# giech/usrp_nfc

Hardware: NVIDIA B200
Metric: decoded_msamples_per_s (higher is better)
Workload: dtype f64

## Files before the change

usrp_nfc_b200/csrc/linecode.cu:

```cuda
#include "common.cuh"
#include "scan.cuh"

#include <algorithm>

namespace nfc {

#ifndef NFC_LC_CHUNK
#define NFC_LC_CHUNK 64
#endif
static const int CHUNK = NFC_LC_CHUNK;
static const int LOOKBACK_LIMIT = 4096;
static const int RSTATES = 32, GSTATES = 16;

struct __align__(16) ChunkMap {
    uint8_t r[RSTATES];
    uint8_t g[GSTATES];
};
struct ComposeMap {
    __device__ __forceinline__ ChunkMap operator()(const ChunkMap &a, const ChunkMap &b) const {
        ChunkMap c;
#pragma unroll
        for (int s = 0; s < RSTATES; s++) c.r[s] = b.r[a.r[s] & 31];
#pragma unroll
        for (int s = 0; s < GSTATES; s++) c.g[s] = b.g[a.g[s] & 15];
// ... 213 lines not shown
    maps[c] = m;
}

struct CountSink {
    ChunkCnt c;
    __device__ __forceinline__ void symbol(uint32_t, int, int) { c.nsym++; }
    __device__ __forceinline__ void emission(uint32_t, int type) {
        uint32_t &has = type == 0 ? c.has0 : c.has1;
        uint32_t &tail = type == 0 ? c.tail0 : c.tail1;
        if (tail != 0) c.nemit++;
        else if (!(has & 1)) { c.nemit++; has |= 2; }
        has |= 1;
        tail = 0;
    }
    __device__ __forceinline__ void bit(int type, int) {
        if (type == 0) { c.nbit0++; c.tail0++; } else { c.nbit1++; c.tail1++; }
    }
    __device__ __forceinline__ void new_capture() {
        c.has0 |= 1; c.tail0 = 0;
        c.has1 |= 1; c.tail1 = 0;
    }
};

__global__ void chunk_summary_kernel(const EventRec *__restrict__ ev, EvCount evc, LineTables lt,
                                     uint16_t *__restrict__ summary) {
    NFC_TABLE_SMEM
    const uint32_t c = blockIdx.x * blockDim.x + threadIdx.x;
    const uint32_t n_ev = evc.n(), n_chunks = (n_ev + CHUNK - 1) / CHUNK;
    if (c >= n_chunks) return;
    int rs = 0, gs = 0;
    bool kR = false, kG = false;
    NullSink sink;
    const uint32_t i0 = c * CHUNK, i1 = min(n_ev, i0 + CHUNK);
    uint32_t cap_prev = tv.pitch ? batch_capture_before(tv, ev, (int64_t)i0) : 0u;
    for (uint32_t i = i0; i < i1; i += 8) {
        EventRec e8[8];
        load8(ev, i, e8);
#pragma unroll
        for (int k = 0; k < 8; k++) {
            if (i + k >= i1) continue;
            const EventRec e = e8[k];
            int dummy = 0;
            if (tv.pitch) {
                bool inside;
                const uint32_t cap = batch_capture(tv, e.rel_pos, inside);
                if (cap != cap_prev) {
// ... 65 lines not shown
                }
                if (!inside) continue;
            }
            if (e.type == 1) {
                if (kk > iR) step_event(e, tv, rs, dummy_g, sink);
            } else if (e.type == 0) {
                if (kk > iG) step_event(e, tv, dummy_r, gs, sink);
            }
        }
    }
    start[c] = (uint16_t)(rs | (gs << 8));
}

__global__ void chunk_start_from_maps_kernel(const ChunkMap *__restrict__ prefix, const DecCarry *__restrict__ carry_in,
                                             uint16_t *__restrict__ start, uint32_t n_chunks) {
    const uint32_t c = blockIdx.x * blockDim.x + threadIdx.x;
    if (c >= n_chunks) return;
    const DecCarry carry = *carry_in;
    const int rs0 = (carry.miller_state & 15) | ((carry.started[1] & 1) << 4);
    const int gs0 = (carry.manch_state & 7) | ((carry.started[0] & 1) << 3);
    start[c] = (uint16_t)(prefix[c].r[rs0] | (prefix[c].g[gs0] << 8));
}

__global__ void chunk_count_kernel(const EventRec *__restrict__ ev, EvCount evc, LineTables lt,
                                   const uint16_t *__restrict__ start, ChunkCnt *__restrict__ cnts, uint32_t cap_chunks) {
    NFC_TABLE_SMEM
    const uint32_t c = blockIdx.x * blockDim.x + threadIdx.x;
    const uint32_t n_ev = evc.n(), n_chunks = (n_ev + CHUNK - 1) / CHUNK;
    if (c >= cap_chunks) return;
    CountSink sink;
    sink.c = ChunkCnt{0, 0, 0, 0, 0, 0, 0, 0};
    if (c >= n_chunks) {
        cnts[c] = sink.c;
        return;
    }
    int rs = start[c] & 31, gs = (start[c] >> 8) & 15;
    const uint32_t i0 = c * CHUNK, i1 = min(n_ev, i0 + CHUNK);
    uint32_t cap_prev = tv.pitch ? batch_capture_before(tv, ev, (int64_t)i0) : 0u;
    for (uint32_t i = i0; i < i1; i += 8) {
        EventRec e[8];
        load8(ev, i, e);
#pragma unroll
        for (int k = 0; k < 8; k++)
            if (i + k < i1) step_event_batch(e[k], tv, rs, gs, sink, cap_prev);
    }
    cnts[c] = sink.c;
}

struct WriteSink {
    SymbolRec *sym;
    uint8_t *bits0, *bits1;
    FrameRec *fr;
    unsigned long long *fx;
    uint32_t *n_empty;
    int64_t a;
    unsigned long long base0, base1;
    uint32_t isym, ib0, ib1, iem;
    uint32_t pend0, pend1;
    uint32_t cap_sym, cap_b0, cap_b1, cap_em;
    __device__ __forceinline__ void symbol(uint32_t pos, int type, int o) {
        if (sym && isym < cap_sym) {
            SymbolRec s;
            s.rel_pos = pos; s.type = (int8_t)type; s.val = (int8_t)o; s.pad = 0;
            sym[isym] = s;
        }
        isym++;
    }
    __device__ __forceinline__ void emission(uint32_t pos, int type) {
        const uint32_t nbits = type == 0 ? pend0 : pend1;
// ... 16 lines not shown
    }
    __device__ __forceinline__ void bit(int type, int o) {
        if (type == 0) { if (ib0 < cap_b0) bits0[ib0] = (uint8_t)o; ib0++; pend0++; }
        else { if (ib1 < cap_b1) bits1[ib1] = (uint8_t)o; ib1++; pend1++; }
    }
    __device__ __forceinline__ void new_capture() { pend0 = 0; pend1 = 0; }
};

struct LineOut {
    SymbolRec *sym;
    uint8_t *bits0, *bits1;
    FrameRec *fr;
    unsigned long long *fx;
    uint32_t cap_sym, cap_b0, cap_b1, cap_em;
    const uint32_t *pending_in;
    int64_t a;
    const unsigned long long *bits_in;
    unsigned long long *bits_out;
    uint32_t *n_empty;
    uint32_t *n_frames;
};

__global__ void chunk_write_kernel(const EventRec *__restrict__ ev, EvCount evc, LineTables lt,
                                   const uint16_t *__restrict__ start,
                                   const ChunkCnt *__restrict__ cnt_prefix, LineOut out, const DecCarry *__restrict__ carry_in,
                                   DecCarry *__restrict__ carry_out, uint32_t *__restrict__ pending_out) {
    NFC_TABLE_SMEM
    const uint32_t c = blockIdx.x * blockDim.x + threadIdx.x;
    const uint32_t n_ev = evc.n(), n_chunks = (n_ev + CHUNK - 1) / CHUNK;
    if (n_chunks == 0 && c == 0) {
        *carry_out = *carry_in;
        pending_out[0] = out.pending_in[0];
        pending_out[1] = out.pending_in[1];
        out.bits_out[0] = out.bits_in[0];
        out.bits_out[1] = out.bits_in[1];
    }
    if (c >= n_chunks) return;
    int rs = start[c] & 31, gs = (start[c] >> 8) & 15;
    const ChunkCnt pc = cnt_prefix[c];
    WriteSink sink;
    sink.sym = out.sym; sink.bits0 = out.bits0; sink.bits1 = out.bits1; sink.fr = out.fr; sink.fx = out.fx;
    sink.n_empty = out.n_empty; sink.a = out.a; sink.base0 = out.bits_in[0]; sink.base1 = out.bits_in[1];
    sink.cap_sym = out.cap_sym; sink.cap_b0 = out.cap_b0; sink.cap_b1 = out.cap_b1; sink.cap_em = out.cap_em;
    sink.isym = pc.nsym; sink.ib0 = pc.nbit0; sink.ib1 = pc.nbit1; sink.iem = resolved_records(pc, out.pending_in);
    sink.pend0 = (pc.has0 & 1) ? pc.tail0 : out.pending_in[0] + pc.tail0;
    sink.pend1 = (pc.has1 & 1) ? pc.tail1 : out.pending_in[1] + pc.tail1;
    const uint32_t i0 = c * CHUNK, i1 = min(n_ev, i0 + CHUNK);
    uint32_t cap_prev = tv.pitch ? batch_capture_before(tv, ev, (int64_t)i0) : 0u;
    for (uint32_t i = i0; i < i1; i += 8) {
        EventRec e[8];
        load8(ev, i, e);
#pragma unroll
        for (int k = 0; k < 8; k++)
            if (i + k < i1) step_event_batch(e[k], tv, rs, gs, sink, cap_prev);
    }
    if (c == n_chunks - 1) {
        DecCarry co;
        co.miller_state = rs & 15; co.started[1] = rs >> 4;
        co.manch_state = gs & 7; co.started[0] = gs >> 3;
        *carry_out = co;
        pending_out[0] = sink.pend0;
        pending_out[1] = sink.pend1;
        out.bits_out[0] = sink.base0 + sink.ib0;
        out.bits_out[1] = sink.base1 + sink.ib1;
        *out.n_frames = sink.iem;
    }
}

uint32_t linecode_chunks(uint32_t n_ev) { return (n_ev + CHUNK - 1) / CHUNK; }
size_t linecode_map_bytes() { return sizeof(ChunkMap); }
size_t linecode_cnt_bytes() { return sizeof(ChunkCnt); }
size_t linecode_emission_bytes() { return sizeof(FrameRec); }
size_t linecode_scratch_bytes(uint32_t n_chunks) {
    return scan_scratch_elems(n_chunks) * sizeof(ChunkMap) + scan_scratch_elems(n_chunks) * sizeof(ChunkCnt);
}

int launch_linecode_start(const EventRec *d_ev, const uint32_t *d_M, uint32_t cap_ev, const LineTables &lt, const DecCarry *d_carry_in,
                          uint16_t *d_summary, uint16_t *d_start, uint32_t *d_flags, cudaStream_t stream) {
    const uint32_t nc = std::max(1u, linecode_chunks(cap_ev));
    const EvCount evc{d_M, cap_ev};
    chunk_summary_kernel<<<(nc + 127) / 128, 128, 0, stream>>>(d_ev, evc, lt, d_summary);
    NFC_CUDA_CHECK(cudaGetLastError());
    chunk_start_kernel<<<(nc + 127) / 128, 128, 0, stream>>>(d_ev, evc, lt, d_carry_in, d_summary, d_start, d_flags);
    NFC_CUDA_CHECK(cudaGetLastError());
    return 0;
}

int launch_linecode_start_scan(const EventRec *d_ev, const uint32_t *d_M, uint32_t cap_ev, const LineTables &lt,
                               const DecCarry *d_carry_in, void *d_maps, void *d_prefix, void *d_scratch, uint16_t *d_start,
                               cudaStream_t stream) {
    const uint32_t nc = std::max(1u, linecode_chunks(cap_ev));
    ChunkMap *maps = (ChunkMap *)d_maps, *prefix = (ChunkMap *)d_prefix;
    const unsigned nb = (nc + 127) / 128;
    const EvCount evc{d_M, cap_ev};
    chunk_map_kernel<<<nb, 128, 0, stream>>>(d_ev, evc, lt, maps, nc);
    NFC_CUDA_CHECK(cudaGetLastError());
    ChunkMap ident;
    for (int s = 0; s < RSTATES; s++) ident.r[s] = (uint8_t)s;
    for (int s = 0; s < GSTATES; s++) ident.g[s] = (uint8_t)s;
    if (device_exclusive_scan<ChunkMap, ComposeMap>(maps, prefix, nc, ident, ComposeMap(), (ChunkMap *)d_scratch, nullptr, stream))
        return -1;
    chunk_start_from_maps_kernel<<<nb, 128, 0, stream>>>(prefix, d_carry_in, d_start, nc);
    NFC_CUDA_CHECK(cudaGetLastError());
    return 0;
}

int launch_linecode_count(const EventRec *d_ev, const uint32_t *d_M, uint32_t cap_ev, const LineTables &lt, const uint16_t *d_start,
                          void *d_cnts, void *d_cnt_prefix, void *d_scratch, void *d_total, cudaStream_t stream) {
    const uint32_t nc = std::max(1u, linecode_chunks(cap_ev));
    ChunkCnt *cnts = (ChunkCnt *)d_cnts, *cprefix = (ChunkCnt *)d_cnt_prefix;
    const EvCount evc{d_M, cap_ev};
    chunk_count_kernel<<<(nc + 127) / 128, 128, 0, stream>>>(d_ev, evc, lt, d_start, cnts, nc);
    NFC_CUDA_CHECK(cudaGetLastError());
    ChunkCnt zero = {0, 0, 0, 0, 0, 0, 0, 0};
    return device_exclusive_scan<ChunkCnt, CombineCnt>(cnts, cprefix, nc, zero, CombineCnt(), (ChunkCnt *)d_scratch,
                                                       (ChunkCnt *)d_total, stream);
}

int launch_linecode_write(const EventRec *d_ev, const uint32_t *d_M, uint32_t cap_ev, const LineTables &lt, const uint16_t *d_start,
                          const void *d_cnt_prefix, SymbolRec *d_sym, uint32_t cap_sym, uint8_t *d_bits0, uint32_t cap_b0,
                          uint8_t *d_bits1, uint32_t cap_b1, void *d_frames, void *d_findex, uint32_t cap_em, int64_t a,
                          const void *d_bits_in, void *d_bits_out, uint32_t *d_n_empty, uint32_t *d_n_frames, const uint32_t *d_pending_in,
                          const DecCarry *d_carry_in, DecCarry *d_carry_out, uint32_t *d_pending_out, cudaStream_t stream) {
    const uint32_t nc = std::max(1u, linecode_chunks(cap_ev));
    LineOut out;
    out.sym = d_sym; out.bits0 = d_bits0; out.bits1 = d_bits1; out.fr = (FrameRec *)d_frames; out.fx = (unsigned long long *)d_findex;
    out.cap_sym = cap_sym; out.cap_b0 = cap_b0; out.cap_b1 = cap_b1; out.cap_em = cap_em;
    out.pending_in = d_pending_in;
    out.a = a;
    out.bits_in = (const unsigned long long *)d_bits_in;
    out.bits_out = (unsigned long long *)d_bits_out;
    out.n_empty = d_n_empty;
    out.n_frames = d_n_frames;
    const EvCount evc{d_M, cap_ev};
    chunk_write_kernel<<<(nc + 127) / 128, 128, 0, stream>>>(d_ev, evc, lt, d_start, (const ChunkCnt *)d_cnt_prefix, out,
                                                             d_carry_in, d_carry_out, d_pending_out);
    NFC_CUDA_CHECK(cudaGetLastError());
    return 0;
}

}
```

usrp_nfc_b200/csrc/runs.cu:

```cuda
#include "common.cuh"
#include "scan.cuh"

namespace nfc {

__global__ void seg_offsets_kernel(const uint32_t *__restrict__ counts, uint32_t *__restrict__ offsets, int n) {
    __shared__ uint32_t sh[1024];
    __shared__ uint32_t carry;
    if (threadIdx.x == 0) carry = 0;
    __syncthreads();
    for (int base = 0; base < n; base += 1024) {
        const int i = base + threadIdx.x;
        uint32_t v = i < n ? counts[i] : 0u;
        sh[threadIdx.x] = v;
        __syncthreads();
        for (int o = 1; o < 1024; o <<= 1) {
            uint32_t a = threadIdx.x >= o ? sh[threadIdx.x - o] : 0u;
            __syncthreads();
            sh[threadIdx.x] += a;
            __syncthreads();
        }
        if (i < n) offsets[i] = carry + sh[threadIdx.x] - v;
        __syncthreads();
        if (threadIdx.x == 1023) carry += sh[1023];
        __syncthreads();
// ... 84 lines not shown
    }
}

struct RunArgs {
    const TransRec *tr;
    const uint32_t *d_R;
    uint32_t cap_R;
    int32_t w0, w1;
    const RunCarry *rc_in;
    int mx;
    uint32_t *flags;
};
__device__ __forceinline__ RunView make_view(const RunArgs &A) {
    RunView V;
    const RunCarry c = *A.rc_in;
    V.tr = A.tr;
    V.R = min(*A.d_R, A.cap_R);
    V.w0 = A.w0; V.w1 = A.w1;
    V.st0 = c.st; V.lb0 = c.last_bit; V.dur0 = c.dur;
    V.mx = A.mx;
    return V;
}

__global__ void run_count_kernel(RunArgs A, int keep_dropped, uint32_t *__restrict__ counts) {
    const uint32_t r = blockIdx.x * blockDim.x + threadIdx.x;
    if (r > A.cap_R) return;
    const RunView V = make_view(A);
    if (r == 0 && *A.d_R > A.cap_R) atomicOr(A.flags, (uint32_t)POST_OVF_TRANS);
    uint32_t c = 0;
    if (r <= V.R) run_events(V, r, keep_dropped != 0, [&](uint32_t, int, int, int) { c++; });
    counts[r] = c;
}

__global__ void run_write_kernel(RunArgs A, int keep_dropped, const uint32_t *__restrict__ offsets,
                                 EventRec *__restrict__ out, uint32_t cap, const uint32_t *__restrict__ d_M,
                                 RunCarry *__restrict__ carry_out) {
    const uint32_t r = blockIdx.x * blockDim.x + threadIdx.x;
    if (r > A.cap_R) return;
    const RunView V = make_view(A);
    if (r == 0 && *d_M > cap) atomicOr(A.flags, (uint32_t)POST_OVF_EVENTS);
    if (r > V.R) return;
    uint32_t idx = offsets[r];
    run_events(V, r, keep_dropped != 0, [&](uint32_t pos, int v, int d, int type) {
        if (idx < cap) {
            EventRec ev;
            ev.rel_pos = pos;
            ev.d = (uint16_t)d;
            ev.v = (int8_t)v;
            ev.type = (int8_t)type;
            out[idx] = ev;
        }
        idx++;
    });
    if (r == V.R && carry_out) {
        RunCarry c;
        if (V.w1 > V.w0) {
            c.st = V.s_end(r);
            c.last_bit = V.u(r);
            c.dur = (int)((uint32_t)(V.w1 - 1 - V.p(r)) % (uint32_t)V.mx) + 1;
        } else {
            c.st = V.st0; c.last_bit = V.lb0; c.dur = V.dur0;
        }
        c.pad = 0;
        *carry_out = c;
    }
}

int launch_gather_transitions(const SegWork *d_works, const uint32_t *d_counts, uint32_t *d_offsets, int n_segs,
                              TransRec *d_dense, cudaStream_t stream) {
    if (n_segs <= 0) return 0;
    seg_offsets_kernel<<<1, 1024, 0, stream>>>(d_counts, d_offsets, n_segs);
    NFC_CUDA_CHECK(cudaGetLastError());
    gather_trans_kernel<<<n_segs, 256, 0, stream>>>(d_works, d_counts, d_offsets, d_dense);
    NFC_CUDA_CHECK(cudaGetLastError());
    return 0;
}

int launch_gather_pieces(const TransRec *const *d_src, const uint32_t *d_n, const uint32_t *d_off, int n_pieces,
                         TransRec *d_dense, cudaStream_t stream) {
    if (n_pieces <= 0) return 0;
    gather_pieces_kernel<<<n_pieces, 256, 0, stream>>>(d_src, d_n, d_off, d_dense);
    NFC_CUDA_CHECK(cudaGetLastError());
    return 0;
}

int launch_run_count(const TransRec *d_tr, const uint32_t *d_R, uint32_t cap_R, int64_t w0, int64_t w1, const RunCarry *d_rc_in,
                     int mx, int keep_dropped, uint32_t *d_counts, uint32_t *d_offsets, uint32_t *d_scratch, uint32_t *d_total,
                     uint32_t *d_flags, cudaStream_t stream) {
    RunArgs A;
    A.tr = d_tr; A.d_R = d_R; A.cap_R = cap_R; A.w0 = (int32_t)w0; A.w1 = (int32_t)w1; A.rc_in = d_rc_in; A.mx = mx; A.flags = d_flags;
    const uint32_t nrun = cap_R + 1;
    run_count_kernel<<<(nrun + 255) / 256, 256, 0, stream>>>(A, keep_dropped, d_counts);
    NFC_CUDA_CHECK(cudaGetLastError());
    return device_exclusive_scan<uint32_t, AddU32>(d_counts, d_offsets, nrun, 0u, AddU32(), d_scratch, d_total, stream);
}

int launch_run_write(const TransRec *d_tr, const uint32_t *d_R, uint32_t cap_R, int64_t w0, int64_t w1, const RunCarry *d_rc_in,
                     int mx, int keep_dropped, const uint32_t *d_offsets, EventRec *d_events, uint32_t cap, const uint32_t *d_M,
                     RunCarry *d_carry_out, uint32_t *d_flags, cudaStream_t stream) {
    RunArgs A;
    A.tr = d_tr; A.d_R = d_R; A.cap_R = cap_R; A.w0 = (int32_t)w0; A.w1 = (int32_t)w1; A.rc_in = d_rc_in; A.mx = mx; A.flags = d_flags;
    const uint32_t nrun = cap_R + 1;
    run_write_kernel<<<(nrun + 255) / 256, 256, 0, stream>>>(A, keep_dropped, d_offsets, d_events, cap, d_M, d_carry_out);
    NFC_CUDA_CHECK(cudaGetLastError());
    return 0;
}

}
```

usrp_nfc_b200/csrc/scan.cuh:

```cuda
#pragma once

#include <cuda_runtime.h>

#include <vector>

#include "common.cuh"

namespace nfc {

static const int SCAN_BLOCK = 256;
static const int SCAN_ITEMS = 4;
static const int SCAN_TILE = SCAN_BLOCK * SCAN_ITEMS;

template <class T>
__device__ __forceinline__ T shfl_up_any(const T &v, int delta) {
    static_assert(sizeof(T) % 4 == 0, "T must be a multiple of 4 bytes");
    T r;
    const unsigned *src = reinterpret_cast<const unsigned *>(&v);
    unsigned *dst = reinterpret_cast<unsigned *>(&r);
#pragma unroll
    for (int i = 0; i < (int)(sizeof(T) / 4); i++) dst[i] = __shfl_up_sync(0xffffffffu, src[i], delta);
    return r;
}

// ... 59 lines not shown

template <class T, class Op>
int device_exclusive_scan(const T *in, T *out, size_t n, T identity, Op op, T *scratch, T *total_out,
                          cudaStream_t stream) {
    if (n == 0) {
        if (total_out) NFC_CUDA_CHECK(cudaMemcpyAsync(total_out, &identity, 0, cudaMemcpyHostToDevice, stream));
        return 0;
    }
    const size_t nb = scan_blocks(n);
    T *totals = scratch;
    T *totals_excl = scratch + nb;
    scan_block_kernel<T, Op><<<(unsigned)nb, SCAN_BLOCK, 0, stream>>>(in, out, totals, n, identity, op);
    NFC_CUDA_CHECK(cudaGetLastError());
    if (nb == 1) {
        if (total_out) NFC_CUDA_CHECK(cudaMemcpyAsync(total_out, totals, sizeof(T), cudaMemcpyDeviceToDevice, stream));
        return 0;
    }
    if (device_exclusive_scan<T, Op>(totals, totals_excl, nb, identity, op, scratch + 2 * nb, total_out, stream)) return -1;
    scan_add_kernel<T, Op><<<(unsigned)nb, SCAN_BLOCK, 0, stream>>>(out, totals_excl, n, op);
    NFC_CUDA_CHECK(cudaGetLastError());
    return 0;
}

struct AddU32 {
    __device__ __forceinline__ uint32_t operator()(uint32_t a, uint32_t b) const { return a + b; }
};

}
```

usrp_nfc_b200/csrc/stream.cu:

```cuda
#include <algorithm>
#include <atomic>
#include <chrono>
#include <cstdarg>
#include <cstdio>
#include <cstdlib>
#include <cstring>
#include <memory>
#include <string>
#include <thread>
#include <deque>
#include <vector>

#include "../../include/usrp_nfc_b200.h"
#include "common.cuh"
#include "tables.h"

namespace nfc {

int launch_slicer(const SegWork *d_works, int n_works, const SlicerParams *d_params, int L, bool vec_ok, cudaStream_t);
bool slicer_streaming_ok(int L, bool vec_ok);
int launch_slicer_streaming(const SegWork *d_works, int n_works, const SlicerParams *d_params, int L, int kind, cudaStream_t);
int launch_extract_count(const uint32_t *d_bm, int64_t bm_pos0, int64_t a, int64_t b, const RunCarry *d_rc_in, int carry_from_bm,
                         uint32_t *d_block_counts, uint32_t *d_block_offsets, uint32_t *d_scan_scratch, uint32_t *d_total,
                         cudaStream_t stream);
int launch_extract_write(const uint32_t *d_bm, int64_t bm_pos0, int64_t a, int64_t b, const RunCarry *d_rc_in, int carry_from_bm,
                         const uint32_t *d_block_offsets, TransRec *d_out, uint32_t out_cap, cudaStream_t stream);
size_t extract_blocks(int64_t bm_pos0, int64_t a, int64_t b);
int launch_slicer_serial(const SegWork *d_works, int n_works, const SlicerParams *d_params, float *d_ring_scratch,
                         size_t ring_stride, cudaStream_t);
int launch_seam_compare(const SlicerHdr *const *d_truth, const SlicerHdr *const *d_assumed, const int *d_param_idx,
                        const SlicerParams *d_params, int *d_mismatch, int n, cudaStream_t);
int launch_gather_transitions(const SegWork *d_works, const uint32_t *d_counts, uint32_t *d_offsets, int n_segs,
                              TransRec *d_dense, cudaStream_t);
int launch_gather_pieces(const TransRec *const *d_src, const uint32_t *d_n, const uint32_t *d_off, int n_pieces,
                         TransRec *d_dense, cudaStream_t);
int launch_run_count(const TransRec *d_tr, const uint32_t *d_R, uint32_t cap_R, int64_t w0, int64_t w1, const RunCarry *d_rc_in,
                     int mx, int keep_dropped, uint32_t *d_counts, uint32_t *d_offsets, uint32_t *d_scratch, uint32_t *d_total,
                     uint32_t *d_flags, cudaStream_t stream);
int launch_run_write(const TransRec *d_tr, const uint32_t *d_R, uint32_t cap_R, int64_t w0, int64_t w1, const RunCarry *d_rc_in,
                     int mx, int keep_dropped, const uint32_t *d_offsets, EventRec *d_events, uint32_t cap, const uint32_t *d_M,
                     RunCarry *d_carry_out, uint32_t *d_flags, cudaStream_t stream);
uint32_t linecode_chunks(uint32_t n_ev);
size_t linecode_map_bytes();
size_t linecode_cnt_bytes();
size_t linecode_emission_bytes();
size_t linecode_scratch_bytes(uint32_t n_chunks);
int launch_linecode_start(const EventRec *d_ev, const uint32_t *d_M, uint32_t cap_ev, const LineTables &lt, const DecCarry *d_carry_in,
                          uint16_t *d_summary, uint16_t *d_start, uint32_t *d_flags, cudaStream_t stream);
int launch_linecode_start_scan(const EventRec *d_ev, const uint32_t *d_M, uint32_t cap_ev, const LineTables &lt,
                               const DecCarry *d_carry_in, void *d_maps, void *d_prefix, void *d_scratch, uint16_t *d_start,
                               cudaStream_t stream);
int launch_linecode_count(const EventRec *d_ev, const uint32_t *d_M, uint32_t cap_ev, const LineTables &lt, const uint16_t *d_start,
                          void *d_cnts, void *d_cnt_prefix, void *d_scratch, void *d_total, cudaStream_t stream);
int launch_linecode_write(const EventRec *d_ev, const uint32_t *d_M, uint32_t cap_ev, const LineTables &lt, const uint16_t *d_start,
                          const void *d_cnt_prefix, SymbolRec *d_sym, uint32_t cap_sym, uint8_t *d_bits0, uint32_t cap_b0,
                          uint8_t *d_bits1, uint32_t cap_b1, void *d_frames, void *d_findex, uint32_t cap_em, int64_t a,
                          const void *d_bits_in, void *d_bits_out, uint32_t *d_n_empty, uint32_t *d_n_frames, const uint32_t *d_pending_in,
                          const DecCarry *d_carry_in, DecCarry *d_carry_out, uint32_t *d_pending_out, cudaStream_t stream);
int slicer_tile(int L, bool vec_ok, int kind);
int slicer_resident_ctas(int L, bool vec_ok, int kind);
int slicer_tile_stats(unsigned long long *out4, bool reset);
int launch_batch_warm(const void *d_items, int64_t stride_bytes, int64_t pitch, int n_cap, int L, const SlicerParams *d_params,
                      void *d_states, size_t state_bytes, cudaStream_t stream);
int launch_bitmap_fill(uint32_t *d_bm, size_t n_chunks, cudaStream_t stream);
int synth_render(void *dev_out, int64_t n, int64_t first_index, const int8_t *codes, const int64_t *lens, int64_t n_runs,
                 float carrier, float pause, float tag_high, float noise, float fade, double fade_period, uint64_t seed,
                 int as_envelope, cudaStream_t);

static thread_local char g_err[512] = "";
void set_error(const char *fmt, ...) {
    va_list ap;
    va_start(ap, fmt);
    vsnprintf(g_err, sizeof(g_err), fmt, ap);
    va_end(ap);
}

struct DevBuf {
    void *p = nullptr;
// ... 114 lines not shown
    cudaEvent_t ev_out[2] = {};
    bool ev_out_set[2] = {false, false};
    DevBuf ctx_d;
    char *ctx_h = nullptr;
    long long slab_seq = 0;
    struct Rates {
        bool have = false;
        double R = 0, M = 0, sym = 0, b0 = 0, b1 = 0, em = 0;
    } rates;

    int64_t pos = 0;
    bool stable = false;
    bool serial_mode = false;
    std::vector<float> warm;
    DevBuf state;
    RunCarry run_carry{0, 0, 0, 0};
    DecCarry dec_carry{0, 0, {0, 0}};
    uint32_t pending[2] = {0, 0};

    int64_t seg_len = 0, halo = 0, slab_len = 0;
    int force_serial = 0;

    DevBuf params_d, tab_d, staging, works_d, states_d, trans_seg, seg_counts, seg_offsets, seg_status,
        seam_ptrs, mismatch_d, run_counts, run_offsets, scan_scr, maps_d, prefix_d, cnts_d, cprefix_d,
        line_scr, serial_ring, start_d, ckpt_d, redo_states, redo_trans,
        redo_counts, pieces_d, bitmap_d, ex_counts, ex_offsets, ex_scr, summ_d;
    DevBuf events_d[2], sym_d[2], bits0_d[2], bits1_d[2], em_d[2], fx_d[2];
    DevBuf trans_dense[2];
    std::vector<DevBuf> kept_bufs;
    static const int NPIN = 3;
    void *pinned[NPIN] = {nullptr, nullptr, nullptr};
    size_t pinned_cap[NPIN] = {0, 0, 0};
    long long slabs_enqueued = 0;
    std::atomic<long long> slabs_marshalled{0};
    std::thread marshal_thr;
    bool blocking_wait = false;
    cudaEvent_t ev_blk = nullptr;
    cudaError_t sync_cs() {
        if (!blocking_wait) return cudaStreamSynchronize(cs);
        const cudaError_t e = cudaEventRecord(ev_blk, cs);
        return e != cudaSuccess ? e : cudaEventSynchronize(ev_blk);
    }
    int set_wait_mode(bool blocking);
    std::atomic<int> marshal_err{0};
    struct SlabJob {
        long long seq = 0;
        int64_t a = 0, b = 0;
// ... 170 lines not shown
    lt.miller = (const TabEntry *)(base + o2);
    lt.manch = (const TabEntry *)(base + o3);
    lt.reset_miller = (const uint8_t *)(base + o4);
    lt.reset_manch = (const uint8_t *)(base + o5);
    lt.n_dclass_miller = ht.n_dclass_miller;
    lt.n_dclass_manch = ht.n_dclass_manch;
    lt.decode_reader = p->decode_reader;
    lt.decode_tag = p->decode_tag;
    lt.batch_pitch = 0;
    lt.batch_skip = 0;
    lt.batch_len = 0;

    warm.reserve((size_t)sp.L);
    if (state.ensure(state_block_bytes(sp.L))) return -1;
    resident_ctas = parallel_ok() ? slicer_resident_ctas(sp.L, vec_ok(), sp.input_kind) : 1;
    if (const char *e = getenv("NFC_SUPER_SLAB")) super_slab = std::max(1, std::min(8, atoi(e)));
    if (const char *e = getenv("NFC_SUPER_BALANCE")) super_balance = atoi(e) != 0;
    return 0;
}

void Stream::destroy() {
    DevBuf *all[] = {&batch_states, &batch_stage, &params_d, &tab_d, &staging, &works_d, &states_d, &trans_seg, &trans_dense[0], &trans_dense[1], &seg_counts, &seg_offsets,
                     &seg_status, &seam_ptrs, &mismatch_d, &run_counts, &run_offsets, &scan_scr, &maps_d,
                     &prefix_d, &cnts_d, &cprefix_d, &line_scr, &ctx_d, &events_d[0], &events_d[1], &sym_d[0], &sym_d[1], &bits0_d[0],
                     &bits0_d[1], &bits1_d[0], &bits1_d[1], &em_d[0], &em_d[1], &fx_d[0], &fx_d[1],
                     &serial_ring, &start_d, &ckpt_d, &redo_states, &redo_trans, &redo_counts, &pieces_d, &state, &bitmap_d,
                     &ex_counts, &ex_offsets, &ex_scr, &summ_d};
    finalize_all();
    if (marshal_thr.joinable()) marshal_thr.join();
    if (cs) cudaStreamSynchronize(cs);
    if (csR) cudaStreamSynchronize(csR);
    if (csL) cudaStreamSynchronize(csL);
    if (cs2) cudaStreamSynchronize(cs2);
    for (DevBuf *b : all) b->release();
    if (ctx_h) cudaFreeHost(ctx_h);
    ctx_h = nullptr;
    fb[0].release();
    fb[1].release();
    out_frames.release();
    findex_drop();
    for (int i = 0; i < NPIN; i++)
        if (pinned[i]) cudaFreeHost(pinned[i]);
    for (int i = 0; i < NCTX; i++) {
        if (ev_a[i]) cudaEventDestroy(ev_a[i]);
        if (ev_b[i]) cudaEventDestroy(ev_b[i]);
        if (ev_c[i]) cudaEventDestroy(ev_c[i]);
        if (ev_ctx[i]) cudaEventDestroy(ev_ctx[i]);
// ... 1006 lines not shown
        if (launch_extract_write(bitmap_d.as<uint32_t>(), bm_origin, a, b, &cp->rc_out, carry_from_bm, ex_offsets.as<uint32_t>(),
                                 td.as<TransRec>(), j.cap_R, cs))
            return -1;
        stats.launches++;
    } else {
        j.cap_R = R_host;
        NFC_CUDA_CHECK(cudaMemcpyAsync(&cx->R, &R_host, 4, cudaMemcpyHostToDevice, cs));
    }
    NFC_CUDA_CHECK(cudaEventRecord(ev_b[ci], cs));
    NFC_CUDA_CHECK(cudaEventRecord(evE[ci], cs));

    NFC_CUDA_CHECK(cudaStreamWaitEvent(csR, evE[ci], 0));
    if (queued(j.seq - 2)) NFC_CUDA_CHECK(cudaStreamWaitEvent(csR, evL[(j.seq - 2) % NCTX], 0));
    if (ev_out_set[oi]) NFC_CUDA_CHECK(cudaStreamWaitEvent(csR, ev_out[oi], 0));
    if (host_events) {
        j.cap_M = n_host_events;
        if (events_d[oi].ensure(((size_t)j.cap_M + 16) * sizeof(EventRec))) return -1;
        if (n_host_events)
            NFC_CUDA_CHECK(cudaMemcpyAsync(events_d[oi].p, host_events, (size_t)n_host_events * sizeof(EventRec), cudaMemcpyHostToDevice, csR));
        NFC_CUDA_CHECK(cudaMemcpyAsync(&cx->M, &n_host_events, 4, cudaMemcpyHostToDevice, csR));
        NFC_CUDA_CHECK(cudaMemcpyAsync(&cx->rc_out, &cp->rc_out, sizeof(RunCarry), cudaMemcpyDeviceToDevice, csR));
        NFC_CUDA_CHECK(cudaStreamSynchronize(csR));
    } else {
    const size_t nrun = (size_t)j.cap_R + 1;
    if (run_counts.ensure(nrun * 4) || run_offsets.ensure(nrun * 4) || scan_scr.ensure((nrun / 256 + 1024) * 4 * 4)) return -1;
    if (launch_run_count(td.as<TransRec>(), &cx->R, j.cap_R, 0, n, &cp->rc_out, sp.mx, keep_dropped, run_counts.as<uint32_t>(),
                         run_offsets.as<uint32_t>(), scan_scr.as<uint32_t>(), &cx->M, &cx->flags, csR))
        return -1;
    stats.launches += 3;
    if (j.exact) {
        uint32_t M = 0;
        NFC_CUDA_CHECK(cudaMemcpyAsync(&M, &cx->M, 4, cudaMemcpyDeviceToHost, csR));
        NFC_CUDA_CHECK(sync_on(csR));
        j.cap_M = M;
    } else {
        j.cap_M = cap_of(rates.M);
    }
    if (events_d[oi].ensure(((size_t)j.cap_M + 16) * sizeof(EventRec))) return -1;
    if (launch_run_write(td.as<TransRec>(), &cx->R, j.cap_R, 0, n, &cp->rc_out, sp.mx, keep_dropped, run_offsets.as<uint32_t>(),
                         events_d[oi].as<EventRec>(), j.cap_M, &cx->M, &cx->rc_out, &cx->flags, csR))
        return -1;
    stats.launches++;
    }
    NFC_CUDA_CHECK(cudaEventRecord(evR[ci], csR));

    NFC_CUDA_CHECK(cudaStreamWaitEvent(csL, evR[ci], 0));
    if (ev_out_set[oi]) NFC_CUDA_CHECK(cudaStreamWaitEvent(csL, ev_out[oi], 0));
    j.have_line = want_line;
    if (want_line) {
        const uint32_t nc = std::max(1u, linecode_chunks(j.cap_M));
        if (start_d.ensure((size_t)nc * 2 + 64) || summ_d.ensure((size_t)nc * 2 + 64) || cnts_d.ensure((size_t)nc * linecode_cnt_bytes()) ||
            cprefix_d.ensure((size_t)nc * linecode_cnt_bytes()) || line_scr.ensure(linecode_scratch_bytes(nc) + 256))
            return -1;
        const EventRec *ev = events_d[oi].as<EventRec>();
        if (launch_linecode_start(ev, &cx->M, j.cap_M, lt, &cp->dc_out, summ_d.as<uint16_t>(), start_d.as<uint16_t>(), &cx->flags, csL)) return -1;
        if (launch_linecode_count(ev, &cx->M, j.cap_M, lt, start_d.as<uint16_t>(), cnts_d.p, cprefix_d.p, line_scr.p, cx->tot, csL)) return -1;
        stats.launches += 6;
        if (j.exact) {
            PostCtx hx;
            NFC_CUDA_CHECK(cudaMemcpyAsync(&hx, cx, 64, cudaMemcpyDeviceToHost, csL));
            NFC_CUDA_CHECK(sync_on(csL));
            if (hx.flags & POST_UNRESOLVED) {
                stats.linecode_scan_fallbacks++;
                if (maps_d.ensure((size_t)nc * linecode_map_bytes()) || prefix_d.ensure((size_t)nc * linecode_map_bytes())) return -1;
                if (launch_linecode_start_scan(ev, &cx->M, j.cap_M, lt, &cp->dc_out, maps_d.p, prefix_d.p, line_scr.p, start_d.as<uint16_t>(), csL))
                    return -1;
                if (launch_linecode_count(ev, &cx->M, j.cap_M, lt, start_d.as<uint16_t>(), cnts_d.p, cprefix_d.p, line_scr.p, cx->tot, csL)) return -1;
                stats.launches += 9;
                NFC_CUDA_CHECK(cudaMemsetAsync(&cx->flags, 0, 4, csL));
                NFC_CUDA_CHECK(cudaMemcpyAsync(&hx, cx, 64, cudaMemcpyDeviceToHost, csL));
                NFC_CUDA_CHECK(sync_on(csL));
            }
            j.cap_sym = hx.tot[0]; j.cap_b0 = hx.tot[1]; j.cap_b1 = hx.tot[2]; j.cap_em = hx.tot[3];
        } else {
            j.cap_sym = cap_of(rates.sym); j.cap_b0 = cap_of(rates.b0); j.cap_b1 = cap_of(rates.b1); j.cap_em = cap_of(rates.em);
        }
        if ((want_sym && sym_d[oi].ensure(((size_t)j.cap_sym + 16) * sizeof(SymbolRec))) || bits0_d[oi].ensure((size_t)j.cap_b0 + 16) ||
            bits1_d[oi].ensure((size_t)j.cap_b1 + 16) || em_d[oi].ensure(((size_t)j.cap_em + 16) * linecode_emission_bytes()) ||
            fx_d[oi].ensure(((size_t)j.cap_em + 16) * 8))
            return -1;
        if (launch_linecode_write(ev, &cx->M, j.cap_M, lt, start_d.as<uint16_t>(), cprefix_d.p, want_sym ? sym_d[oi].as<SymbolRec>() : nullptr,
                                  want_sym ? j.cap_sym : 0, bits0_d[oi].as<uint8_t>(), j.cap_b0, bits1_d[oi].as<uint8_t>(), j.cap_b1, em_d[oi].p,
                                  fx_d[oi].p, j.cap_em, a, cp->bits_out, cx->bits_out, &cx->n_empty, &cx->n_frames, cp->pend_out, &cp->dc_out, &cx->dc_out,
                                  cx->pend_out, csL))
            return -1;
        stats.launches++;
    } else {
        NFC_CUDA_CHECK(cudaMemcpyAsync(&cx->dc_out, &cp->dc_out, sizeof(DecCarry) + 8 + 8 + 16, cudaMemcpyDeviceToDevice, csL));
    }
    NFC_CUDA_CHECK(cudaEventRecord(ev_c[ci], csL));
    NFC_CUDA_CHECK(cudaMemcpyAsync(ctx_h + (size_t)ci * 256, cx, 256, cudaMemcpyDeviceToHost, csL));
    NFC_CUDA_CHECK(cudaEventRecord(ev_ctx[ci], csL));
    NFC_CUDA_CHECK(cudaEventRecord(evL[ci], csL));
    j.want_ev = (prm.outputs & NFC_OUT_EVENTS) != 0;
    j.want_sym = want_sym && want_line;
    j.want_fr = (prm.outputs & NFC_OUT_FRAMES) != 0 && want_line;
    j.t2 = now_ms();
    jobs.push_back(j);
    while (jobs.size() > 1)
        if (finalize_front()) return -1;
    return 0;
}

int Stream::settle_frames() {
// ... 675 lines not shown
```

Measured before the change: 473,300.

## Replace per-element device scans with block-level reductions plus in-kernel block prefix

The run count and line-code count kernels now reduce each thread block to a single total, and only the per-block totals go through the multi-pass device scan. The write kernels rebuild each element's offset with an in-block warp-shuffle scan added to the block prefix. This shrinks the scan input by the block size, which can remove scan launches and global traffic for the per-element counts and prefix arrays. In exchange, run_write now recomputes each run's event count and both write kernels do an extra block-wide scan with a __syncthreads.

```diff
diff --git a/usrp_nfc_b200/csrc/linecode.cu b/usrp_nfc_b200/csrc/linecode.cu
--- a/usrp_nfc_b200/csrc/linecode.cu
+++ b/usrp_nfc_b200/csrc/linecode.cu
@@ -259,6 +259,32 @@
     }
 };
 
+static const int LC_BLOCK = 128;
+__device__ __forceinline__ ChunkCnt block_exclusive_cnt(const ChunkCnt &v, ChunkCnt *total) {
+    __shared__ ChunkCnt wtot[LC_BLOCK / 32];
+    const CombineCnt op;
+    const ChunkCnt zero = {0, 0, 0, 0, 0, 0, 0, 0};
+    const int lane = threadIdx.x & 31, warp = threadIdx.x >> 5;
+    ChunkCnt inc = v;
+#pragma unroll
+    for (int o = 1; o < 32; o <<= 1) {
+        const ChunkCnt nb = shfl_up_any(inc, o);
+        if (lane >= o) inc = op(nb, inc);
+    }
+    ChunkCnt exc = shfl_up_any(inc, 1);
+    if (lane == 0) exc = zero;
+    if (lane == 31) wtot[warp] = inc;
+    __syncthreads();
+    ChunkCnt wbase = zero, tot = zero;
+#pragma unroll
+    for (int w = 0; w < LC_BLOCK / 32; w++) {
+        if (w < warp) wbase = op(wbase, wtot[w]);
+        tot = op(tot, wtot[w]);
+    }
+    if (total) *total = tot;
+    return op(wbase, exc);
+}
+
 __global__ void chunk_summary_kernel(const EventRec *__restrict__ ev, EvCount evc, LineTables lt,
                                      uint16_t *__restrict__ summary) {
     NFC_TABLE_SMEM
@@ -370,29 +396,30 @@
     start[c] = (uint16_t)(prefix[c].r[rs0] | (prefix[c].g[gs0] << 8));
 }
 
-__global__ void chunk_count_kernel(const EventRec *__restrict__ ev, EvCount evc, LineTables lt,
-                                   const uint16_t *__restrict__ start, ChunkCnt *__restrict__ cnts, uint32_t cap_chunks) {
+__global__ void __launch_bounds__(LC_BLOCK) chunk_count_kernel(const EventRec *__restrict__ ev, EvCount evc, LineTables lt,
+                                                               const uint16_t *__restrict__ start, ChunkCnt *__restrict__ cnts,
+                                                               ChunkCnt *__restrict__ block_cnts, uint32_t cap_chunks) {
     NFC_TABLE_SMEM
     const uint32_t c = blockIdx.x * blockDim.x + threadIdx.x;
     const uint32_t n_ev = evc.n(), n_chunks = (n_ev + CHUNK - 1) / CHUNK;
-    if (c >= cap_chunks) return;
     CountSink sink;
     sink.c = ChunkCnt{0, 0, 0, 0, 0, 0, 0, 0};
-    if (c >= n_chunks) {
-        cnts[c] = sink.c;
-        return;
-    }
-    int rs = start[c] & 31, gs = (start[c] >> 8) & 15;
-    const uint32_t i0 = c * CHUNK, i1 = min(n_ev, i0 + CHUNK);
-    uint32_t cap_prev = tv.pitch ? batch_capture_before(tv, ev, (int64_t)i0) : 0u;
-    for (uint32_t i = i0; i < i1; i += 8) {
-        EventRec e[8];
-        load8(ev, i, e);
-#pragma unroll
-        for (int k = 0; k < 8; k++)
-            if (i + k < i1) step_event_batch(e[k], tv, rs, gs, sink, cap_prev);
-    }
-    cnts[c] = sink.c;
+    if (c < n_chunks) {
+        int rs = start[c] & 31, gs = (start[c] >> 8) & 15;
+        const uint32_t i0 = c * CHUNK, i1 = min(n_ev, i0 + CHUNK);
+        uint32_t cap_prev = tv.pitch ? batch_capture_before(tv, ev, (int64_t)i0) : 0u;
+        for (uint32_t i = i0; i < i1; i += 8) {
+            EventRec e[8];
+            load8(ev, i, e);
+#pragma unroll
+            for (int k = 0; k < 8; k++)
+                if (i + k < i1) step_event_batch(e[k], tv, rs, gs, sink, cap_prev);
+        }
+    }
+    if (c < cap_chunks) cnts[c] = sink.c;
+    ChunkCnt tot;
+    block_exclusive_cnt(sink.c, &tot);
+    if (threadIdx.x == 0) block_cnts[blockIdx.x] = tot;
 }
 
 struct WriteSink {
@@ -455,12 +482,15 @@
 };
 
 __global__ void chunk_write_kernel(const EventRec *__restrict__ ev, EvCount evc, LineTables lt,
-                                   const uint16_t *__restrict__ start,
-                                   const ChunkCnt *__restrict__ cnt_prefix, LineOut out, const DecCarry *__restrict__ carry_in,
-                                   DecCarry *__restrict__ carry_out, uint32_t *__restrict__ pending_out) {
+                                   const uint16_t *__restrict__ start, const ChunkCnt *__restrict__ cnts,
+                                   const ChunkCnt *__restrict__ block_prefix, uint32_t cap_chunks, LineOut out,
+                                   const DecCarry *__restrict__ carry_in, DecCarry *__restrict__ carry_out,
+                                   uint32_t *__restrict__ pending_out) {
     NFC_TABLE_SMEM
     const uint32_t c = blockIdx.x * blockDim.x + threadIdx.x;
     const uint32_t n_ev = evc.n(), n_chunks = (n_ev + CHUNK - 1) / CHUNK;
+    const ChunkCnt zero = {0, 0, 0, 0, 0, 0, 0, 0};
+    const ChunkCnt in_block = block_exclusive_cnt(c < cap_chunks ? cnts[c] : zero, nullptr);
     if (n_chunks == 0 && c == 0) {
         *carry_out = *carry_in;
         pending_out[0] = out.pending_in[0];
@@ -470,7 +500,7 @@
     }
     if (c >= n_chunks) return;
     int rs = start[c] & 31, gs = (start[c] >> 8) & 15;
-    const ChunkCnt pc = cnt_prefix[c];
+    const ChunkCnt pc = CombineCnt()(block_prefix[blockIdx.x], in_block);
     WriteSink sink;
     sink.sym = out.sym; sink.bits0 = out.bits0; sink.bits1 = out.bits1; sink.fr = out.fr; sink.fx = out.fx;
     sink.n_empty = out.n_empty; sink.a = out.a; sink.base0 = out.bits_in[0]; sink.base1 = out.bits_in[1];
@@ -502,11 +532,16 @@
 
 uint32_t linecode_chunks(uint32_t n_ev) { return (n_ev + CHUNK - 1) / CHUNK; }
 size_t linecode_map_bytes() { return sizeof(ChunkMap); }
-size_t linecode_cnt_bytes() { return sizeof(ChunkCnt); }
 size_t linecode_emission_bytes() { return sizeof(FrameRec); }
 size_t linecode_scratch_bytes(uint32_t n_chunks) {
     return scan_scratch_elems(n_chunks) * sizeof(ChunkMap) + scan_scratch_elems(n_chunks) * sizeof(ChunkCnt);
 }
+static inline uint32_t linecode_blocks(uint32_t cap_ev) { return (std::max(1u, linecode_chunks(cap_ev)) + LC_BLOCK - 1) / LC_BLOCK; }
+size_t linecode_cnt_buffer_bytes(uint32_t cap_ev) {
+    return ((size_t)linecode_blocks(cap_ev) * LC_BLOCK + 2 * (size_t)linecode_blocks(cap_ev)) * sizeof(ChunkCnt);
+}
+int linecode_count_launches(uint32_t cap_ev) { return 1 + scan_launches(linecode_blocks(cap_ev)); }
+int linecode_start_scan_launches(uint32_t cap_ev) { return 2 + scan_launches(std::max(1u, linecode_chunks(cap_ev))); }
 
 int launch_linecode_start(const EventRec *d_ev, const uint32_t *d_M, uint32_t cap_ev, const LineTables &lt, const DecCarry *d_carry_in,
                           uint16_t *d_summary, uint16_t *d_start, uint32_t *d_flags, cudaStream_t stream) {
@@ -539,23 +574,24 @@
 }
 
 int launch_linecode_count(const EventRec *d_ev, const uint32_t *d_M, uint32_t cap_ev, const LineTables &lt, const uint16_t *d_start,
-                          void *d_cnts, void *d_cnt_prefix, void *d_scratch, void *d_total, cudaStream_t stream) {
-    const uint32_t nc = std::max(1u, linecode_chunks(cap_ev));
-    ChunkCnt *cnts = (ChunkCnt *)d_cnts, *cprefix = (ChunkCnt *)d_cnt_prefix;
+                          void *d_cnts, void *d_scratch, void *d_total, cudaStream_t stream) {
+    const uint32_t nc = std::max(1u, linecode_chunks(cap_ev)), nb = linecode_blocks(cap_ev);
+    ChunkCnt *cnts = (ChunkCnt *)d_cnts, *btot = cnts + (size_t)nb * LC_BLOCK, *bprefix = btot + nb;
     const EvCount evc{d_M, cap_ev};
-    chunk_count_kernel<<<(nc + 127) / 128, 128, 0, stream>>>(d_ev, evc, lt, d_start, cnts, nc);
+    chunk_count_kernel<<<nb, LC_BLOCK, 0, stream>>>(d_ev, evc, lt, d_start, cnts, btot, nc);
     NFC_CUDA_CHECK(cudaGetLastError());
     ChunkCnt zero = {0, 0, 0, 0, 0, 0, 0, 0};
-    return device_exclusive_scan<ChunkCnt, CombineCnt>(cnts, cprefix, nc, zero, CombineCnt(), (ChunkCnt *)d_scratch,
+    return device_exclusive_scan<ChunkCnt, CombineCnt>(btot, bprefix, nb, zero, CombineCnt(), (ChunkCnt *)d_scratch,
                                                        (ChunkCnt *)d_total, stream);
 }
 
 int launch_linecode_write(const EventRec *d_ev, const uint32_t *d_M, uint32_t cap_ev, const LineTables &lt, const uint16_t *d_start,
-                          const void *d_cnt_prefix, SymbolRec *d_sym, uint32_t cap_sym, uint8_t *d_bits0, uint32_t cap_b0,
+                          const void *d_cnts, SymbolRec *d_sym, uint32_t cap_sym, uint8_t *d_bits0, uint32_t cap_b0,
                           uint8_t *d_bits1, uint32_t cap_b1, void *d_frames, void *d_findex, uint32_t cap_em, int64_t a,
                           const void *d_bits_in, void *d_bits_out, uint32_t *d_n_empty, uint32_t *d_n_frames, const uint32_t *d_pending_in,
                           const DecCarry *d_carry_in, DecCarry *d_carry_out, uint32_t *d_pending_out, cudaStream_t stream) {
-    const uint32_t nc = std::max(1u, linecode_chunks(cap_ev));
+    const uint32_t nc = std::max(1u, linecode_chunks(cap_ev)), nb = linecode_blocks(cap_ev);
+    const ChunkCnt *cnts = (const ChunkCnt *)d_cnts, *bprefix = cnts + (size_t)nb * LC_BLOCK + nb;
     LineOut out;
     out.sym = d_sym; out.bits0 = d_bits0; out.bits1 = d_bits1; out.fr = (FrameRec *)d_frames; out.fx = (unsigned long long *)d_findex;
     out.cap_sym = cap_sym; out.cap_b0 = cap_b0; out.cap_b1 = cap_b1; out.cap_em = cap_em;
@@ -566,8 +602,8 @@
     out.n_empty = d_n_empty;
     out.n_frames = d_n_frames;
     const EvCount evc{d_M, cap_ev};
-    chunk_write_kernel<<<(nc + 127) / 128, 128, 0, stream>>>(d_ev, evc, lt, d_start, (const ChunkCnt *)d_cnt_prefix, out,
-                                                             d_carry_in, d_carry_out, d_pending_out);
+    chunk_write_kernel<<<nb, LC_BLOCK, 0, stream>>>(d_ev, evc, lt, d_start, cnts, bprefix, nc, out, d_carry_in, d_carry_out,
+                                                    d_pending_out);
     NFC_CUDA_CHECK(cudaGetLastError());
     return 0;
 }
diff --git a/usrp_nfc_b200/csrc/runs.cu b/usrp_nfc_b200/csrc/runs.cu
--- a/usrp_nfc_b200/csrc/runs.cu
+++ b/usrp_nfc_b200/csrc/runs.cu
@@ -130,26 +130,55 @@
     return V;
 }
 
-__global__ void run_count_kernel(RunArgs A, int keep_dropped, uint32_t *__restrict__ counts) {
-    const uint32_t r = blockIdx.x * blockDim.x + threadIdx.x;
-    if (r > A.cap_R) return;
+static const int RUN_BLOCK = 256;
+
+__device__ __forceinline__ uint32_t run_count(const RunView &V, uint32_t r, int keep_dropped) {
+    uint32_t c = 0;
+    if (r <= V.R) run_events(V, r, keep_dropped != 0, [&](uint32_t, int, int, int) { c++; });
+    return c;
+}
+
+__global__ void __launch_bounds__(RUN_BLOCK) run_count_kernel(RunArgs A, int keep_dropped, uint32_t *__restrict__ block_counts) {
+    const uint32_t r = blockIdx.x * RUN_BLOCK + threadIdx.x;
     const RunView V = make_view(A);
     if (r == 0 && *A.d_R > A.cap_R) atomicOr(A.flags, (uint32_t)POST_OVF_TRANS);
-    uint32_t c = 0;
-    if (r <= V.R) run_events(V, r, keep_dropped != 0, [&](uint32_t, int, int, int) { c++; });
-    counts[r] = c;
-}
-
-__global__ void run_write_kernel(RunArgs A, int keep_dropped, const uint32_t *__restrict__ offsets,
-                                 EventRec *__restrict__ out, uint32_t cap, const uint32_t *__restrict__ d_M,
-                                 RunCarry *__restrict__ carry_out) {
-    const uint32_t r = blockIdx.x * blockDim.x + threadIdx.x;
-    if (r > A.cap_R) return;
+    const uint32_t c = run_count(V, r, keep_dropped);
+    __shared__ uint32_t wsum[RUN_BLOCK / 32];
+    const uint32_t s = __reduce_add_sync(0xffffffffu, c);
+    if ((threadIdx.x & 31) == 0) wsum[threadIdx.x >> 5] = s;
+    __syncthreads();
+    if (threadIdx.x == 0) {
+        uint32_t t = 0;
+#pragma unroll
+        for (int q = 0; q < RUN_BLOCK / 32; q++) t += wsum[q];
+        block_counts[blockIdx.x] = t;
+    }
+}
+
+__global__ void __launch_bounds__(RUN_BLOCK) run_write_kernel(RunArgs A, int keep_dropped, const uint32_t *__restrict__ block_offsets,
+                                                              EventRec *__restrict__ out, uint32_t cap, const uint32_t *__restrict__ d_M,
+                                                              RunCarry *__restrict__ carry_out) {
+    const uint32_t r = blockIdx.x * RUN_BLOCK + threadIdx.x;
     const RunView V = make_view(A);
     if (r == 0 && *d_M > cap) atomicOr(A.flags, (uint32_t)POST_OVF_EVENTS);
+    const uint32_t c = run_count(V, r, keep_dropped);
+    const int lane = threadIdx.x & 31, warp = threadIdx.x >> 5;
+    uint32_t inc = c;
+#pragma unroll
+    for (int o = 1; o < 32; o <<= 1) {
+        const uint32_t v = __shfl_up_sync(0xffffffffu, inc, o);
+        if (lane >= o) inc += v;
+    }
+    __shared__ uint32_t wsum[RUN_BLOCK / 32];
+    if (lane == 31) wsum[warp] = inc;
+    __syncthreads();
+    uint32_t wbase = 0;
+#pragma unroll
+    for (int q = 0; q < RUN_BLOCK / 32; q++)
+        if (q < warp) wbase += wsum[q];
     if (r > V.R) return;
-    uint32_t idx = offsets[r];
-    run_events(V, r, keep_dropped != 0, [&](uint32_t pos, int v, int d, int type) {
+    uint32_t idx = block_offsets[blockIdx.x] + wbase + inc - c;
+    if (c) run_events(V, r, keep_dropped != 0, [&](uint32_t pos, int v, int d, int type) {
         if (idx < cap) {
             EventRec ev;
             ev.rel_pos = pos;
@@ -161,16 +190,16 @@
         idx++;
     });
     if (r == V.R && carry_out) {
-        RunCarry c;
+        RunCarry co;
         if (V.w1 > V.w0) {
-            c.st = V.s_end(r);
-            c.last_bit = V.u(r);
-            c.dur = (int)((uint32_t)(V.w1 - 1 - V.p(r)) % (uint32_t)V.mx) + 1;
+            co.st = V.s_end(r);
+            co.last_bit = V.u(r);
+            co.dur = (int)((uint32_t)(V.w1 - 1 - V.p(r)) % (uint32_t)V.mx) + 1;
         } else {
-            c.st = V.st0; c.last_bit = V.lb0; c.dur = V.dur0;
-        }
-        c.pad = 0;
-        *carry_out = c;
+            co.st = V.st0; co.last_bit = V.lb0; co.dur = V.dur0;
+        }
+        co.pad = 0;
+        *carry_out = co;
     }
 }
 
@@ -192,24 +221,27 @@
     return 0;
 }
 
+static inline uint32_t run_blocks(uint32_t cap_R) { return (uint32_t)(((uint64_t)cap_R + 1 + RUN_BLOCK - 1) / RUN_BLOCK); }
+size_t run_count_blocks(uint32_t cap_R) { return run_blocks(cap_R); }
+int run_count_launches(uint32_t cap_R) { return 1 + scan_launches(run_blocks(cap_R)); }
+
 int launch_run_count(const TransRec *d_tr, const uint32_t *d_R, uint32_t cap_R, int64_t w0, int64_t w1, const RunCarry *d_rc_in,
-                     int mx, int keep_dropped, uint32_t *d_counts, uint32_t *d_offsets, uint32_t *d_scratch, uint32_t *d_total,
+                     int mx, int keep_dropped, uint32_t *d_block_counts, uint32_t *d_block_offsets, uint32_t *d_scratch, uint32_t *d_total,
                      uint32_t *d_flags, cudaStream_t stream) {
     RunArgs A;
     A.tr = d_tr; A.d_R = d_R; A.cap_R = cap_R; A.w0 = (int32_t)w0; A.w1 = (int32_t)w1; A.rc_in = d_rc_in; A.mx = mx; A.flags = d_flags;
-    const uint32_t nrun = cap_R + 1;
-    run_count_kernel<<<(nrun + 255) / 256, 256, 0, stream>>>(A, keep_dropped, d_counts);
-    NFC_CUDA_CHECK(cudaGetLastError());
-    return device_exclusive_scan<uint32_t, AddU32>(d_counts, d_offsets, nrun, 0u, AddU32(), d_scratch, d_total, stream);
+    const uint32_t nblk = run_blocks(cap_R);
+    run_count_kernel<<<nblk, RUN_BLOCK, 0, stream>>>(A, keep_dropped, d_block_counts);
+    NFC_CUDA_CHECK(cudaGetLastError());
+    return device_exclusive_scan<uint32_t, AddU32>(d_block_counts, d_block_offsets, nblk, 0u, AddU32(), d_scratch, d_total, stream);
 }
 
 int launch_run_write(const TransRec *d_tr, const uint32_t *d_R, uint32_t cap_R, int64_t w0, int64_t w1, const RunCarry *d_rc_in,
-                     int mx, int keep_dropped, const uint32_t *d_offsets, EventRec *d_events, uint32_t cap, const uint32_t *d_M,
+                     int mx, int keep_dropped, const uint32_t *d_block_offsets, EventRec *d_events, uint32_t cap, const uint32_t *d_M,
                      RunCarry *d_carry_out, uint32_t *d_flags, cudaStream_t stream) {
     RunArgs A;
     A.tr = d_tr; A.d_R = d_R; A.cap_R = cap_R; A.w0 = (int32_t)w0; A.w1 = (int32_t)w1; A.rc_in = d_rc_in; A.mx = mx; A.flags = d_flags;
-    const uint32_t nrun = cap_R + 1;
-    run_write_kernel<<<(nrun + 255) / 256, 256, 0, stream>>>(A, keep_dropped, d_offsets, d_events, cap, d_M, d_carry_out);
+    run_write_kernel<<<run_blocks(cap_R), RUN_BLOCK, 0, stream>>>(A, keep_dropped, d_block_offsets, d_events, cap, d_M, d_carry_out);
     NFC_CUDA_CHECK(cudaGetLastError());
     return 0;
 }
diff --git a/usrp_nfc_b200/csrc/scan.cuh b/usrp_nfc_b200/csrc/scan.cuh
--- a/usrp_nfc_b200/csrc/scan.cuh
+++ b/usrp_nfc_b200/csrc/scan.cuh
@@ -105,6 +105,12 @@
     return 0;
 }
 
+static inline int scan_launches(size_t n) {
+    if (n == 0) return 0;
+    const size_t nb = scan_blocks(n);
+    return nb == 1 ? 1 : 2 + scan_launches(nb);
+}
+
 struct AddU32 {
     __device__ __forceinline__ uint32_t operator()(uint32_t a, uint32_t b) const { return a + b; }
 };
diff --git a/usrp_nfc_b200/csrc/stream.cu b/usrp_nfc_b200/csrc/stream.cu
--- a/usrp_nfc_b200/csrc/stream.cu
+++ b/usrp_nfc_b200/csrc/stream.cu
@@ -40,9 +40,13 @@
 int launch_run_write(const TransRec *d_tr, const uint32_t *d_R, uint32_t cap_R, int64_t w0, int64_t w1, const RunCarry *d_rc_in,
                      int mx, int keep_dropped, const uint32_t *d_offsets, EventRec *d_events, uint32_t cap, const uint32_t *d_M,
                      RunCarry *d_carry_out, uint32_t *d_flags, cudaStream_t stream);
+size_t run_count_blocks(uint32_t cap_R);
+int run_count_launches(uint32_t cap_R);
 uint32_t linecode_chunks(uint32_t n_ev);
 size_t linecode_map_bytes();
-size_t linecode_cnt_bytes();
+size_t linecode_cnt_buffer_bytes(uint32_t cap_ev);
+int linecode_count_launches(uint32_t cap_ev);
+int linecode_start_scan_launches(uint32_t cap_ev);
 size_t linecode_emission_bytes();
 size_t linecode_scratch_bytes(uint32_t n_chunks);
 int launch_linecode_start(const EventRec *d_ev, const uint32_t *d_M, uint32_t cap_ev, const LineTables &lt, const DecCarry *d_carry_in,
@@ -51,9 +55,9 @@
                                const DecCarry *d_carry_in, void *d_maps, void *d_prefix, void *d_scratch, uint16_t *d_start,
                                cudaStream_t stream);
 int launch_linecode_count(const EventRec *d_ev, const uint32_t *d_M, uint32_t cap_ev, const LineTables &lt, const uint16_t *d_start,
-                          void *d_cnts, void *d_cnt_prefix, void *d_scratch, void *d_total, cudaStream_t stream);
+                          void *d_cnts, void *d_scratch, void *d_total, cudaStream_t stream);
 int launch_linecode_write(const EventRec *d_ev, const uint32_t *d_M, uint32_t cap_ev, const LineTables &lt, const uint16_t *d_start,
-                          const void *d_cnt_prefix, SymbolRec *d_sym, uint32_t cap_sym, uint8_t *d_bits0, uint32_t cap_b0,
+                          const void *d_cnts, SymbolRec *d_sym, uint32_t cap_sym, uint8_t *d_bits0, uint32_t cap_b0,
                           uint8_t *d_bits1, uint32_t cap_b1, void *d_frames, void *d_findex, uint32_t cap_em, int64_t a,
                           const void *d_bits_in, void *d_bits_out, uint32_t *d_n_empty, uint32_t *d_n_frames, const uint32_t *d_pending_in,
                           const DecCarry *d_carry_in, DecCarry *d_carry_out, uint32_t *d_pending_out, cudaStream_t stream);
@@ -214,7 +218,7 @@
     int force_serial = 0;
 
     DevBuf params_d, tab_d, staging, works_d, states_d, trans_seg, seg_counts, seg_offsets, seg_status,
-        seam_ptrs, mismatch_d, run_counts, run_offsets, scan_scr, maps_d, prefix_d, cnts_d, cprefix_d,
+        seam_ptrs, mismatch_d, run_counts, run_offsets, scan_scr, maps_d, prefix_d, cnts_d,
         line_scr, serial_ring, start_d, ckpt_d, redo_states, redo_trans,
         redo_counts, pieces_d, bitmap_d, ex_counts, ex_offsets, ex_scr, summ_d;
     DevBuf events_d[2], sym_d[2], bits0_d[2], bits1_d[2], em_d[2], fx_d[2];
@@ -431,7 +435,7 @@
 void Stream::destroy() {
     DevBuf *all[] = {&batch_states, &batch_stage, &params_d, &tab_d, &staging, &works_d, &states_d, &trans_seg, &trans_dense[0], &trans_dense[1], &seg_counts, &seg_offsets,
                      &seg_status, &seam_ptrs, &mismatch_d, &run_counts, &run_offsets, &scan_scr, &maps_d,
-                     &prefix_d, &cnts_d, &cprefix_d, &line_scr, &ctx_d, &events_d[0], &events_d[1], &sym_d[0], &sym_d[1], &bits0_d[0],
+                     &prefix_d, &cnts_d, &line_scr, &ctx_d, &events_d[0], &events_d[1], &sym_d[0], &sym_d[1], &bits0_d[0],
                      &bits0_d[1], &bits1_d[0], &bits1_d[1], &em_d[0], &em_d[1], &fx_d[0], &fx_d[1],
                      &serial_ring, &start_d, &ckpt_d, &redo_states, &redo_trans, &redo_counts, &pieces_d, &state, &bitmap_d,
                      &ex_counts, &ex_offsets, &ex_scr, &summ_d};
@@ -1484,12 +1488,12 @@
         NFC_CUDA_CHECK(cudaMemcpyAsync(&cx->rc_out, &cp->rc_out, sizeof(RunCarry), cudaMemcpyDeviceToDevice, csR));
         NFC_CUDA_CHECK(cudaStreamSynchronize(csR));
     } else {
-    const size_t nrun = (size_t)j.cap_R + 1;
-    if (run_counts.ensure(nrun * 4) || run_offsets.ensure(nrun * 4) || scan_scr.ensure((nrun / 256 + 1024) * 4 * 4)) return -1;
+    const size_t nrblk = run_count_blocks(j.cap_R);
+    if (run_counts.ensure((nrblk + 16) * 4) || run_offsets.ensure((nrblk + 16) * 4) || scan_scr.ensure((nrblk / 256 + 1024) * 4 * 4)) return -1;
     if (launch_run_count(td.as<TransRec>(), &cx->R, j.cap_R, 0, n, &cp->rc_out, sp.mx, keep_dropped, run_counts.as<uint32_t>(),
                          run_offsets.as<uint32_t>(), scan_scr.as<uint32_t>(), &cx->M, &cx->flags, csR))
         return -1;
-    stats.launches += 3;
+    stats.launches += run_count_launches(j.cap_R);
     if (j.exact) {
         uint32_t M = 0;
         NFC_CUDA_CHECK(cudaMemcpyAsync(&M, &cx->M, 4, cudaMemcpyDeviceToHost, csR));
@@ -1511,13 +1515,13 @@
     j.have_line = want_line;
     if (want_line) {
         const uint32_t nc = std::max(1u, linecode_chunks(j.cap_M));
-        if (start_d.ensure((size_t)nc * 2 + 64) || summ_d.ensure((size_t)nc * 2 + 64) || cnts_d.ensure((size_t)nc * linecode_cnt_bytes()) ||
-            cprefix_d.ensure((size_t)nc * linecode_cnt_bytes()) || line_scr.ensure(linecode_scratch_bytes(nc) + 256))
+        if (start_d.ensure((size_t)nc * 2 + 64) || summ_d.ensure((size_t)nc * 2 + 64) || cnts_d.ensure(linecode_cnt_buffer_bytes(j.cap_M)) ||
+            line_scr.ensure(linecode_scratch_bytes(nc) + 256))
             return -1;
         const EventRec *ev = events_d[oi].as<EventRec>();
         if (launch_linecode_start(ev, &cx->M, j.cap_M, lt, &cp->dc_out, summ_d.as<uint16_t>(), start_d.as<uint16_t>(), &cx->flags, csL)) return -1;
-        if (launch_linecode_count(ev, &cx->M, j.cap_M, lt, start_d.as<uint16_t>(), cnts_d.p, cprefix_d.p, line_scr.p, cx->tot, csL)) return -1;
-        stats.launches += 6;
+        if (launch_linecode_count(ev, &cx->M, j.cap_M, lt, start_d.as<uint16_t>(), cnts_d.p, line_scr.p, cx->tot, csL)) return -1;
+        stats.launches += 2 + linecode_count_launches(j.cap_M);
         if (j.exact) {
             PostCtx hx;
             NFC_CUDA_CHECK(cudaMemcpyAsync(&hx, cx, 64, cudaMemcpyDeviceToHost, csL));
@@ -1527,8 +1531,8 @@
                 if (maps_d.ensure((size_t)nc * linecode_map_bytes()) || prefix_d.ensure((size_t)nc * linecode_map_bytes())) return -1;
                 if (launch_linecode_start_scan(ev, &cx->M, j.cap_M, lt, &cp->dc_out, maps_d.p, prefix_d.p, line_scr.p, start_d.as<uint16_t>(), csL))
                     return -1;
-                if (launch_linecode_count(ev, &cx->M, j.cap_M, lt, start_d.as<uint16_t>(), cnts_d.p, cprefix_d.p, line_scr.p, cx->tot, csL)) return -1;
-                stats.launches += 9;
+                if (launch_linecode_count(ev, &cx->M, j.cap_M, lt, start_d.as<uint16_t>(), cnts_d.p, line_scr.p, cx->tot, csL)) return -1;
+                stats.launches += linecode_start_scan_launches(j.cap_M) + linecode_count_launches(j.cap_M);
                 NFC_CUDA_CHECK(cudaMemsetAsync(&cx->flags, 0, 4, csL));
                 NFC_CUDA_CHECK(cudaMemcpyAsync(&hx, cx, 64, cudaMemcpyDeviceToHost, csL));
                 NFC_CUDA_CHECK(sync_on(csL));
@@ -1541,7 +1545,7 @@
             bits1_d[oi].ensure((size_t)j.cap_b1 + 16) || em_d[oi].ensure(((size_t)j.cap_em + 16) * linecode_emission_bytes()) ||
             fx_d[oi].ensure(((size_t)j.cap_em + 16) * 8))
             return -1;
-        if (launch_linecode_write(ev, &cx->M, j.cap_M, lt, start_d.as<uint16_t>(), cprefix_d.p, want_sym ? sym_d[oi].as<SymbolRec>() : nullptr,
+        if (launch_linecode_write(ev, &cx->M, j.cap_M, lt, start_d.as<uint16_t>(), cnts_d.p, want_sym ? sym_d[oi].as<SymbolRec>() : nullptr,
                                   want_sym ? j.cap_sym : 0, bits0_d[oi].as<uint8_t>(), j.cap_b0, bits1_d[oi].as<uint8_t>(), j.cap_b1, em_d[oi].p,
                                   fx_d[oi].p, j.cap_em, a, cp->bits_out, cx->bits_out, &cx->n_empty, &cx->n_frames, cp->pend_out, &cp->dc_out, &cx->dc_out,
                                   cx->pend_out, csL))
```

After: 468,600 (median of 6 runs). -1.0%, worse.
